# ReadAlongs/SoundSwallower

Hardware: AMD Instinct MI355X
Metric: senone-frames/sec (en-us PTM) (higher is better)
Workload: dtype f32+i32

## Files before the change

soundswallower_amd/csrc/ssw_host_active.inc:

```

static int
active_first_frames(const int32_t *sf, const int32_t *ef, int n_phones, int n_frames,
                    std::vector<int32_t> &first)
{
    first.assign((size_t)n_phones, INT_MAX);
    int32_t prev_first = 0, prev_last = 0;
    for (int i = 0; i < n_phones; ++i) {
        if (i > 0 && (sf[i] < sf[i - 1] || ef[i] < ef[i - 1])) {
            ssw_set_error("ssw_align_batch_active: phone windows must not decrease along an "
                          "utterance (phone %d); with such windows the reference's active set "
                          "depends on the path scores", i);
            return -1;
        }
        int32_t fi = i == 0 ? 0 : std::max(std::max((int32_t)1, sf[i]), prev_first);
        if (i > 0 && fi > prev_last)
            break;
        if (fi >= n_frames)
            break;
        first[i] = fi;
        prev_first = fi;
        prev_last = ef[i] < fi ? fi : ef[i];
    }
    return 0;
}
// ... 198 lines not shown
align_batch_active_impl(ssw_model_t *m, int scorer, const float *d_feats, int32_t n_utts,
                        const int32_t *frame_off, const int32_t *phone_off, const uint16_t *senid,
                        const int16_t *tmatid, const int32_t *sf, const int32_t *ef,
                        const uint32_t *seed_active, ssw_align_entry_t *state_io, int32_t *status,
                        int16_t *d_senscr, void *stream, const uint32_t *d_carry_rows)
{
    ModelBusy busy_(m);
    if (!busy_.ok)
        return -1;
    const ssw_host_model_t *h = m->h;
    hipStream_t st = (hipStream_t)stream;
    if (semi_refuse(scorer, "ssw_align_batch_active") < 0
        || cont_refuse(m, "ssw_align_batch_active") < 0)
        return -1;
    if (n_utts <= 0)
        return 0;
    if (check_scorer_shape(m, scorer) < 0)
        return -1;
    if (h->n_cb > 64 || h->n_emit_state != 3) {
        ssw_set_error("ssw_align_batch_active: built for <= 64 codebooks and 3-state HMMs");
        return -1;
    }
    if (h->cfg.ds != 1 || m->force_exact) {
        ssw_set_error("active-set batches: ds = 1 only");
        return -1;
    }
    if (!d_feats || !frame_off || !phone_off || !senid || !tmatid || !sf || !ef || !state_io
        || !status || frame_off[0] != 0 || phone_off[0] != 0) {
        ssw_set_error("ssw_align_batch_active: bad arguments");
        return -1;
    }
    HIP_OK(hipSetDevice(m->device));
    const int n_frames = frame_off[n_utts];
    std::vector<uint16_t> sen_slot((size_t)h->n_sen, 0);
    {
        std::vector<int> next((size_t)h->n_cb + 1, 0);
        for (int i = 0; i < h->n_sen; ++i)
            ++next[(size_t)h->sen2cb[i] + 1];
        for (int c = 0; c < h->n_cb; ++c)
            next[(size_t)c + 1] = next[(size_t)c] + ((next[(size_t)c + 1] + 3) & ~3);
        for (int i = 0; i < h->n_sen; ++i)
            sen_slot[(size_t)i] = (uint16_t)next[(size_t)h->sen2cb[i]]++;
    }
    std::vector<ActiveUtt> per_utt((size_t)n_utts);
    {
        ActiveJob J;
        J.h = h;
        J.sen_slot = sen_slot.data();
        J.n_utts = n_utts;
        J.frame_off = frame_off;
        J.phone_off = phone_off;
        J.sf = sf;
        J.ef = ef;
        J.senid = senid;
        J.seed_active = seed_active;
        J.out = per_utt.data();
        J.per_chunk = std::max(1, (n_utts + 4 * ssw_host_threads() - 1) / (4 * ssw_host_threads()));
        ssw_parallel_for((n_utts + J.per_chunk - 1) / J.per_chunk, active_build_chunk, &J);
    }
    std::vector<int32_t> seg_of_frame((size_t)std::max(n_frames, 1));
    std::vector<int32_t> seg_utt, seg_nreal, seg_boff(1, 0), utt_real_off((size_t)n_utts + 1, 0);
    std::vector<uint32_t> real_ent, bridge_ent;
    std::vector<uint16_t> real_rank;
    std::vector<unsigned long long> seg_cbmask;
    int cap = 1;
    for (int u = 0; u < n_utts; ++u) {
        const ActiveUtt &A = per_utt[(size_t)u];
        if (A.err != 0) {
            ssw_set_error("%s", A.msg);
            return -1;
        }
        const int f0 = frame_off[u], nf = frame_off[u + 1] - f0;
        utt_real_off[(size_t)u] = (int32_t)real_ent.size();
        real_ent.insert(real_ent.end(), A.real_ent.begin(), A.real_ent.end());
        real_rank.insert(real_rank.end(), A.real_rank.begin(), A.real_rank.end());
        utt_real_off[(size_t)u + 1] = (int32_t)real_ent.size();
        bridge_ent.insert(bridge_ent.end(), A.bridge_ent.begin(), A.bridge_ent.end());
        cap = std::max(cap, A.cap);
        for (size_t k = 0; k < A.seg_start.size(); ++k) {
            const int seg = (int)seg_utt.size();
            const int t0 = A.seg_start[k], t1 = k + 1 < A.seg_start.size() ? A.seg_start[k + 1] : nf;
// ... 86 lines not shown
```

soundswallower_amd/csrc/ssw_host_model.inc:

```

struct Knobs {
    int sen_fpb;
    int sen_r;
    int sen_groups;
    bool sen_generic;
    bool ms_senone_old;
    bool scan_fma;
    int mfma_min_frames;
    int score_piece;
    int host_pipe_cap;
    int mfma_steps;
    bool mfma_balance;
    int mfma_lds_pad;
    bool ptm_exact;
    bool frame_fused;
    int scan_audit;
    float selftest_eps_u;
    bool selftest_off;
    bool align_band, align_win;
    bool align_bt;
    char align_kernel[8];
    int align_band_tokens;
    int align_win_waves;
    bool align_timing;
    bool fp_band, fp_win;
    char fp_kernel[8];
    int fp_hist_band;
    int fp_big_tpb, fp_win_tpb;
    int fpa_sub;
};

static bool
knobs_dynamic()
{
    static const bool dyn = [] {
        const char *e = getenv("SSW_KNOBS_DYNAMIC");
        return e != NULL && e[0] == '1';
    }();
    return dyn;
}

static void
load_knobs(Knobs &k)
{
    auto env_int = [](const char *name, int dflt) {
        const char *e = getenv(name);
        return e != NULL ? atoi(e) : dflt;
    };
    auto env_is = [](const char *name, const char *val) {
        const char *e = getenv(name);
        return e != NULL && strcmp(e, val) == 0;
    };
    const char *e;
    e = getenv("SSW_SEN_FPB");
    k.sen_fpb = (e != NULL && (e[0] == '1' || e[0] == '2')) ? e[0] - '0' : 0;
    e = getenv("SSW_SEN_R");
    k.sen_r = (e != NULL && e[0] >= '1' && e[0] <= '4') ? e[0] - '0' : 0;
    e = getenv("SSW_SEN_GROUPS");
    k.sen_groups = e != NULL ? (atoi(e) > 0 ? atoi(e) : 0) : -1;
    k.sen_generic = getenv("SSW_SEN_GENERIC") != NULL;
    k.ms_senone_old = env_is("SSW_MS_SENONE", "old");
    k.scan_fma = env_is("SSW_SCAN", "fma");
    k.mfma_min_frames = env_int("SSW_MFMA_MIN_FRAMES", 1);
    k.fpa_sub = env_int("SSW_FPA_SUB", -1);
    k.score_piece = env_int("SSW_SCORE_PIECE", 16384) / 256 * 256;
    k.host_pipe_cap = std::max(2, env_int("SSW_HOST_PIPE_CAP", 16384) & ~1);
    e = getenv("SSW_MFMA_STEPS");
    k.mfma_steps = e != NULL ? (e[0] == '2' ? 2 : 1) : 0;
    e = getenv("SSW_MFMA_BALANCE");
    k.mfma_balance = !(e != NULL && e[0] == '0');
    k.mfma_lds_pad = env_int("SSW_MFMA_LDS_PAD", 0);
    e = getenv("SSW_PTM_EXACT");
    k.ptm_exact = e != NULL && e[0] == '1';
    k.frame_fused = getenv("SSW_FRAME_FUSED") != NULL;
    k.scan_audit = env_int("SSW_SCAN_AUDIT", 0);
    if (k.scan_audit < 0)
        k.scan_audit = 0;
    e = getenv("SSW_MFMA_SELFTEST_EPS");
    k.selftest_eps_u = e != NULL ? (float)atof(e) : 34.0f;
    k.selftest_off = env_is("SSW_MFMA_SELFTEST", "off");
    auto env_not0 = [](const char *name) {
        const char *v = getenv(name);
        return !(v != NULL && v[0] == '0');
    };
    auto env_str = [](const char *name, char (&dst)[8]) {
        const char *v = getenv(name);
        snprintf(dst, sizeof(dst), "%s", v != NULL ? v : "");
    };
    k.align_band = env_not0("SSW_ALIGN_BAND");
    k.align_win = env_not0("SSW_ALIGN_WIN");
    k.align_bt = env_not0("SSW_ALIGN_BT");
    env_str("SSW_ALIGN_KERNEL", k.align_kernel);
    k.align_band_tokens = env_int("SSW_ALIGN_BAND_TOKENS", 0);
// ... 47 lines not shown
    hipEvent_t ev[3];
    hipEvent_t ev_sc;

    uint32_t *cw() const { return topn_cw.as<uint32_t>(); }
    int4 *sc() const { return topn_sc.as<int4>(); }
    int *utt_off() const { return meta.as<int>(); }
    uint32_t *utt_start() const { return meta.as<uint32_t>() + ws_utts; }
};

struct ssw_model_s {
    ssw_host_model_t *h;
    Knobs kn;
    int scan_mode;
    int selftest_status;
    float selftest_worst_u, selftest_ms;
    char selftest_msg[200];
    int device;
    int n_cu;
    std::atomic<unsigned long long> owner;
    int owner_depth;
    int n_cbf, sen_stride;
    float *d_rec;
    float *d_rec28;
    float *d_recq;
    float *d_recmax;
    uint32_t *d_exlist;
    uint4 *d_wfrag;
    uint32_t *d_exlistm;
    int n_exact_form;
    uint8_t *d_mixw, *d_ms_pdf, *d_sen2cb, *d_logadd8, *d_logadd_mirror, *d_tp, *d_quad_cb;
    short4 *d_slot_sen;
    uint32_t *d_quad_info;
    uint16_t *d_sen_slot;
    DevBuf act_ws;
    int n_quads, slot_stride;
    int logadd_max;
    ScoreWs sw;
    DevBuf carry0;
    DevBuf carry_rows;
    unsigned char *h_stage[2];
    size_t h_stage_cap[2];
    hipEvent_t ev_stage[2];
    int stage_next;
    hipStream_t s_pipe, s_copy;
    hipEvent_t ev_piece[2], ev_down[2];
    unsigned char *h_pipe_feat[2], *h_pipe_out[2];
    float *d_pipe_feat[2];
    int16_t *d_pipe_out[2];
    size_t pipe_feat_cap, pipe_out_cap;
    int force_exact;
    int ms_raw;
    int64_t align_stats[2];
    int align_state_out_only;
    DevBuf feat_off;
    ssw_fe_tables_t *d_fe_tab;
    ssw_fe_config_t fe_tab_cfg;
    std::map<std::string, ssw_fe_rate_t *> *fe_rate_tab;
    int fe_nfilt, fe_noise;
    DevBuf fe_ws;
    hipEvent_t fe_ev[4];
    int fe_ev_ready, fe_timed;
    DevBuf align_ws;
    DevBuf fp_ws;
    hipStream_t s_up;
    hipEvent_t ev_up;
    uint64_t fp_ws_uid;
// ... 241 lines not shown
            HIP_OK(hipMemcpy(m->d_rec28, h->rec28, (size_t)ncbf * h->n_density * 28 * sizeof(float),
                             hipMemcpyHostToDevice));
            HIP_OK(hipMemcpy(m->d_exlistm, h->exlistm, nex * sizeof(uint32_t),
                             hipMemcpyHostToDevice));
        }
    }
    HIP_OK(hipMalloc((void **)&m->d_logadd8, 256));
    HIP_OK(hipMemcpy(m->d_logadd8, h->logadd8, 256, hipMemcpyHostToDevice));
    {
        int T = 0;
        for (int i = 0; i < 256; ++i)
            T = h->logadd8[i] > T ? h->logadd8[i] : T;
        m->logadd_max = T;
        std::vector<uint8_t> mir((size_t)3 * SSW_LOGADD_MIRROR);
        for (int part = 0; part < 2; ++part) {
            const int size = (part + 1) * SSW_LOGADD_MIRROR, mid = size / 2;
            uint8_t *out = mir.data() + (part ? SSW_LOGADD_MIRROR : 0);
            for (int e = 0; e < size; ++e) {
                const int d = e < mid ? mid - e : e - mid;
                out[e] = (uint8_t)(T - (d < 256 ? (int)h->logadd8[d] : 0));
            }
        }
        HIP_OK(hipMalloc((void **)&m->d_logadd_mirror, mir.size()));
        HIP_OK(hipMemcpy(m->d_logadd_mirror, mir.data(), mir.size(), hipMemcpyHostToDevice));
    }
    if (h->n_sen && h->sen2cb != NULL && h->cont_rec == NULL) {
        std::vector<uint8_t> s2c((size_t)h->n_sen);
        for (int i = 0; i < h->n_sen; ++i)
            s2c[i] = (uint8_t)h->sen2cb[i];
        HIP_OK(hipMalloc((void **)&m->d_sen2cb, s2c.size()));
        HIP_OK(hipMemcpy(m->d_sen2cb, s2c.data(), s2c.size(), hipMemcpyHostToDevice));
    }
    if ((h->ptm_mixw || h->ms_pdf) && h->sc_rec == NULL && h->cont_rec == NULL) {
        std::vector<int16_t> slot_sen;
        std::vector<uint8_t> quad_cb;
        for (int c = 0; c < h->n_cb; ++c) {
            size_t start = slot_sen.size();
            for (int i = 0; i < h->n_sen; ++i)
                if (h->sen2cb[i] == c)
                    slot_sen.push_back((int16_t)i);
            while ((slot_sen.size() - start) % 4)
                slot_sen.push_back(-1);
            for (size_t q = start / 4; q < slot_sen.size() / 4; ++q)
                quad_cb.push_back((uint8_t)c);
        }
        m->n_quads = (int)quad_cb.size();
        m->slot_stride = ((int)slot_sen.size() + 127) & ~127;
        m->sen_stride = m->slot_stride;
        const size_t rows = (size_t)h->n_feat * h->n_density;
        if (h->ptm_mixw) {
            std::vector<uint8_t> mw(rows * m->slot_stride, 0);
            for (size_t r = 0; r < rows; ++r)
                for (size_t sl = 0; sl < slot_sen.size(); ++sl) {
                    const int sen = slot_sen[sl] >= 0 ? slot_sen[sl] : slot_sen[sl & ~(size_t)3];
                    mw[r * m->slot_stride + sl] = h->ptm_mixw[r * h->n_sen + sen];
                }
            HIP_OK(hipMalloc((void **)&m->d_mixw, mw.size()));
            HIP_OK(hipMemcpy(m->d_mixw, mw.data(), mw.size(), hipMemcpyHostToDevice));
        }
        if (h->ms_pdf) {
            std::vector<uint8_t> mw(rows * m->slot_stride, 0);
            for (size_t sl = 0; sl < slot_sen.size(); ++sl) {
                const int sen = slot_sen[sl] >= 0 ? slot_sen[sl] : slot_sen[sl & ~(size_t)3];
                const uint8_t *src = h->ms_pdf + (size_t)sen * rows;
                for (size_t r = 0; r < rows; ++r)
                    mw[r * m->slot_stride + sl] = src[r];
            }
            HIP_OK(hipMalloc((void **)&m->d_ms_pdf, mw.size()));
            HIP_OK(hipMemcpy(m->d_ms_pdf, mw.data(), mw.size(), hipMemcpyHostToDevice));
        }
        {
            std::vector<uint32_t> qi(quad_cb.size());
            for (size_t q = 0; q < qi.size(); ++q) {
                const int16_t *sj = &slot_sen[4 * q];
                const bool run4 = sj[0] >= 0 && sj[1] == sj[0] + 1 && sj[2] == sj[0] + 2
                    && sj[3] == sj[0] + 3;
                qi[q] = ((uint32_t)sj[0] & 0xffffu) | ((uint32_t)run4 << 16)
                    | ((uint32_t)quad_cb[q] << 24);
            }
            HIP_OK(hipMalloc((void **)&m->d_quad_info, qi.size() * sizeof(uint32_t)));
            HIP_OK(hipMemcpy(m->d_quad_info, qi.data(), qi.size() * sizeof(uint32_t),
                             hipMemcpyHostToDevice));
        }
        HIP_OK(hipMalloc((void **)&m->d_quad_cb, quad_cb.size()));
        HIP_OK(hipMemcpy(m->d_quad_cb, quad_cb.data(), quad_cb.size(), hipMemcpyHostToDevice));
        {
            std::vector<uint16_t> sen_slot((size_t)h->n_sen, 0);
            for (size_t sl = 0; sl < slot_sen.size(); ++sl)
                if (slot_sen[sl] >= 0)
                    sen_slot[(size_t)slot_sen[sl]] = (uint16_t)sl;
            HIP_OK(hipMalloc((void **)&m->d_sen_slot, sen_slot.size() * sizeof(uint16_t) + 16));
            HIP_OK(hipMemcpy(m->d_sen_slot, sen_slot.data(), sen_slot.size() * sizeof(uint16_t),
                             hipMemcpyHostToDevice));
        }
        HIP_OK(hipMalloc((void **)&m->d_slot_sen, slot_sen.size() * sizeof(int16_t)));
        HIP_OK(hipMemcpy(m->d_slot_sen, slot_sen.data(), slot_sen.size() * sizeof(int16_t),
                         hipMemcpyHostToDevice));
    }
    if (h->tp) {
        size_t n = (size_t)h->tp_n_tmat * h->tp_n_state * (h->tp_n_state + 1);
        HIP_OK(hipMalloc((void **)&m->d_tp, n + 16));
        HIP_OK(hipMemcpy(m->d_tp, h->tp, n, hipMemcpyHostToDevice));
    }
    return 0;
}

static void
mfma_self_test(ssw_model_s *m)
{
    m->scan_mode = m->d_wfrag != NULL ? 1 : 0;
    m->selftest_status = 0;
    m->selftest_msg[0] = 0;
    if (m->d_wfrag == NULL || m->kn.selftest_off)
        return;
    {
        void *sym = NULL;
        if (hipGetSymbolAddress(&sym, HIP_SYMBOL(g_selftest_out)) != hipSuccess)
            (void)hipGetLastError();
    }
    const auto t0 = std::chrono::steady_clock::now();
    std::vector<float2> out((size_t)SSW_SELFTEST_TILES);
    hipLaunchKernelGGL(mfma_selftest_kernel, dim3(SSW_SELFTEST_TILES), dim3(64), 0, 0, 0x5eed2026u);
    hipError_t e = hipGetLastError();
    if (e == hipSuccess)
        e = hipMemcpyFromSymbol(out.data(), HIP_SYMBOL(g_selftest_out), sizeof(float2) * out.size());
    const float eps = m->kn.selftest_eps_u;
// ... 101 lines not shown
{
    if (m == NULL)
        return;
    ssw_feat_free(m->own_feat);
    if (m->device == SSW_DEVICE_NONE) {
        ssw_host_model_free(m->h);
        delete m;
        return;
    }
    (void)hipFree(m->featex_ws.p);
    (void)hipFree(m->d_rec);
    (void)hipFree(m->d_rec28);
    (void)hipFree(m->d_recq);
    (void)hipFree(m->d_recmax);
    (void)hipFree(m->d_exlist);
    (void)hipFree(m->d_wfrag);
    (void)hipFree(m->d_exlistm);
    (void)hipFree(m->align_ws.p);
    (void)hipFree(m->fp_ws.p);
    (void)hipFree(m->fpa_ws.p);
    (void)hipFree(m->gr_ws.p);
    (void)hipFree(m->text_scr.p);
    (void)hipFree(m->feat_off.p);
    (void)hipFree(m->d_fe_tab);
    if (m->fe_rate_tab)
        for (auto &kv : *m->fe_rate_tab)
            (void)hipFree(kv.second);
    delete m->fe_rate_tab;
    (void)hipFree(m->fe_ws.p);
    if (m->fe_ev_ready)
        for (int i = 0; i < 4; ++i)
            (void)hipEventDestroy(m->fe_ev[i]);
    (void)hipFree(m->d_sen_slot);
    (void)hipFree(m->act_ws.p);
    (void)hipFree(m->d_mixw);
    (void)hipFree(m->d_ms_pdf);
    (void)hipFree(m->d_sen2cb);
    if (m->s_up) {
        (void)hipEventDestroy(m->ev_up);
        (void)hipStreamDestroy(m->s_up);
    }
    (void)hipFree(m->d_quad_cb);
    (void)hipFree(m->d_quad_info);
    (void)hipFree(m->d_slot_sen);
    (void)hipFree(m->d_logadd8);
    (void)hipFree(m->d_logadd_mirror);
    (void)hipFree(m->d_tp);
    (void)hipFree(m->sw.topn_cw.p);
    (void)hipFree(m->sw.topn_sc.p);
    (void)hipFree(m->sw.meta.p);
    (void)hipFree(m->carry0.p);
    (void)hipFree(m->carry_rows.p);
    (void)hipFree(m->sw.d_nfixed);
    delete m->sw.utt_cache;
    delete m->sw.xcd_cuts;
    for (int k = 0; k < 2; ++k) {
        if (m->h_stage[k] != NULL) {
            (void)hipHostFree(m->h_stage[k]);
            (void)hipEventDestroy(m->ev_stage[k]);
        }
    }
    if (m->s_copy != NULL) {
        (void)hipStreamDestroy(m->s_copy);
        (void)hipStreamDestroy(m->s_pipe);
        for (int k = 0; k < 2; ++k) {
            (void)hipEventDestroy(m->ev_piece[k]);
// ... 119 lines not shown
```

soundswallower_amd/csrc/ssw_host_score.inc:

```
static int
ensure_score_ws(ssw_model_s *m, size_t rows, int n_utts)
{
    ScoreWs &w = m->sw;
    const uint64_t pairs = (uint64_t)rows * (uint64_t)m->n_cbf;
    if (pairs > 0xffffffffull) {
        ssw_set_error("batch of %d frames is too large (frames x codebooks x streams must fit 32 bits)",
                      (int)rows);
        return -1;
    }
    if (devbuf_reserve(w.topn_cw, sizeof(uint32_t) * (size_t)pairs, "ssw_score_batch") < 0
        || devbuf_reserve(w.topn_sc, sizeof(int4) * (size_t)pairs, "ssw_score_batch") < 0)
        return -1;
    if (w.d_nfixed == NULL) {
        if (dev_alloc(&w.d_nfixed, 4) < 0)
            return -1;
        HIP_OK(hipMemset(w.d_nfixed, 0, 4 * sizeof(unsigned long long)));
    }
    const size_t need_bits = 2 * ((rows + 31) / 32 + 2);
    if ((size_t)n_utts + 1 > w.ws_utts || need_bits > w.ws_bits) {
        const size_t wu = std::max((size_t)n_utts + 1, w.ws_utts_hint), wb = std::max(need_bits, w.ws_bits_hint);
        bool moved = false;
        w.ws_utts = w.ws_bits = 0;
        const int rc = devbuf_reserve(w.meta, sizeof(uint32_t) * (wu + wb), "ssw_score_batch", 0, &moved);
        if (moved && w.utt_cache)
// ... 129 lines not shown
    S.quad_info = m->d_quad_info;
    S.slot_sen = m->d_slot_sen;
    S.logadd8 = m->d_logadd8;
    S.logadd_mirror = m->d_logadd_mirror + (scorer == SSW_SCORER_MS ? SSW_LOGADD_MIRROR : 0);
    S.nfixed = move_stats ? m->sw.d_nfixed : NULL;
    S.nfixed_acc = m->sw.stats_accumulate;
    S.out = cp != NULL ? C.R.d_out : C.R.d_out + (size_t)lo * h->n_sen;
    if (cp != NULL) {
        S.utt_of_frame = cp->d_utt_of_frame;
        S.cutt_off = cp->d_frame_off;
        S.cstride = cp->d_cstride;
        S.crow_off = cp->d_crow_off;
        S.cpos = cp->d_cpos;
        S.frame_base = lo;
    }
    S.n_frames = n_frames;
    S.n_cb = h->n_cb;
    S.n_feat = h->n_feat;
    S.n_density = h->n_density;
    S.n_sen = h->n_sen;
    S.slot_stride = m->slot_stride;
    S.n_quads = m->n_quads;
    S.tab_max = m->logadd_max;
    if (scorer != SSW_SCORER_MS && 255 + SSW_MAX_NEG_ASCR + 3 * S.tab_max >= SSW_LOGADD_LDS) {
        ssw_set_error("unsupported log-add table (largest entry %d)", S.tab_max);
        return -1;
    }
    const bool ptm = scorer != SSW_SCORER_MS;
    const Knobs &kn = m->kn;
    int fpb = n_frames >= 4 * 512 ? 2 : 1;
    if (kn.sen_fpb != 0 && n_frames >= 4 * 512)
        fpb = kn.sen_fpb;
    size_t lds = 0;
    int R = (m->n_quads + SEN_MAX_THREADS - 1) / SEN_MAX_THREADS;
    const bool ms_packed = !ptm && ms_takes_packed_kernel(m, n_frames);
    if (cp != NULL && !ptm && !ms_packed) {
        ssw_set_error("internal error: compact rows asked of the un-packed ms senone kernel");
        return -1;
    }
    if ((ptm || ms_packed) && fpb == 2 && R < 4) {
        const int r7 = (m->n_quads + 447) / 448;
        R = r7 > R ? (r7 > 4 ? 4 : r7) : R;
    }
    if (kn.sen_r != 0)
        R = kn.sen_r;
    int threads = ((m->n_quads + R - 1) / R + 63) & ~63;
    if (threads < 256)
        threads = 256;
    if (threads > SEN_MAX_THREADS || (scorer == SSW_SCORER_MS && threads < m->n_cbf)) {
        ssw_set_error("unsupported senone/codebook shape (%d quads, %d codebook x stream)",
                      m->n_quads, m->n_cbf);
        return -1;
    }
    if (scorer == SSW_SCORER_MS && !ms_packed) {
        lds = 256 + 20 * (size_t)m->n_cbf + 16 * sizeof(int);
#define SSW_MS_LAUNCH(RR)                                                                    \
    if (h->n_feat == 3 && !kn.sen_generic)                                                   \
        hipLaunchKernelGGL((ms_senone_kernel<RR, 3>), dim3(n_frames), dim3(threads), lds, st, S); \
    else                                                                                     \
        hipLaunchKernelGGL((ms_senone_kernel<RR, 0>), dim3(n_frames), dim3(threads), lds, st, S)
        switch (R) {
        case 1: SSW_MS_LAUNCH(1); break;
        case 2: SSW_MS_LAUNCH(2); break;
        case 3: SSW_MS_LAUNCH(3); break;
        case 4: SSW_MS_LAUNCH(4); break;
        default:
            ssw_set_error("too many senones (%d quads)", m->n_quads);
            return -1;
        }
#undef SSW_MS_LAUNCH
        HIP_OK(hipGetLastError());
        return 0;
    }
    if (threads < fpb * m->n_cbf)
        fpb = 1;
    if (threads < m->n_cbf) {
        ssw_set_error("unsupported senone/codebook shape (%d quads, %d codebook x stream)",
                      m->n_quads, m->n_cbf);
        return -1;
    }
    lds = (ms_packed ? 2 * SSW_LOGADD_MIRROR : SSW_LOGADD_MIRROR)
        + 3 * 4 * (size_t)(ms_packed ? ((h->n_cb + 7) & ~7) : SSW_MAX_FEAT) * fpb + 16 * sizeof(int)
        + 2 * 32 * (size_t)m->n_cbf * fpb
        + 20 * (size_t)((fpb * m->n_cbf + 63) & ~63)
        + 8 * (size_t)R * threads + 16;
    const int n_units = (n_frames + fpb - 1) / fpb;
    int per_cu = 32 / (threads / 64);
    per_cu = per_cu < 1 ? 1 : per_cu;
    int groups = m->n_cu * per_cu;
    if ((C.R.flags & SSW_SCORE_SHARE_DEVICE) != 0 && groups < (n_units + 7) / 8)
        groups = (n_units + 7) / 8;
    if (kn.sen_groups >= 0)
        groups = kn.sen_groups > 0 ? kn.sen_groups : n_units;
    const dim3 grid(groups < n_units ? groups : n_units);
    const bool nf3 = h->n_feat == 3 && !kn.sen_generic;
    if (fpb != 1 && fpb != 2) {
        ssw_set_error("senone kernel: %d frames per group (1 or 2)", fpb);
        return -1;
    }
#define SSW_SEN_LAUNCH_C(RR, FP, NFV, MSV, CV)                                               \
    hipLaunchKernelGGL((ptm_senone_kernel<4, RR, FP, NFV, MSV, CV>), grid, dim3(threads), lds, st, S)
#define SSW_SEN_LAUNCH_NF(RR, FP, MSV, CV)                                                   \
    if (nf3)                                                                                 \
        SSW_SEN_LAUNCH_C(RR, FP, 3, MSV, CV);                                                \
    else                                                                                     \
        SSW_SEN_LAUNCH_C(RR, FP, 0, MSV, CV)
#define SSW_SEN_LAUNCH_FP(RR, MSV, CV)                                                       \
    if (fpb == 2) {                                                                          \
        SSW_SEN_LAUNCH_NF(RR, 2, MSV, CV);                                                   \
    } else {                                                                                 \
        SSW_SEN_LAUNCH_NF(RR, 1, MSV, CV);                                                   \
    }
#define SSW_SEN_LAUNCH(RR)                                                                   \
    if (ms_packed && cp != NULL) {                                                           \
        SSW_SEN_LAUNCH_FP(RR, true, true);                                                   \
    } else if (ms_packed) {                                                                  \
        SSW_SEN_LAUNCH_FP(RR, true, false);                                                  \
    } else if (cp != NULL) {                                                                 \
// ... 937 lines not shown
```

soundswallower_amd/csrc/ssw_k1b_senone.inc:

```

struct SenoneParams {
    const uint32_t *topn_cw;
    const int4 *topn_sc;
    const uint8_t *mixw;
    const uint8_t *quad_cb;
    const short4 *slot_sen;
    const uint32_t *quad_info;
    const uint8_t *logadd8;
    const uint8_t *logadd_mirror;
    unsigned long long *nfixed;
    int16_t *out;
    int n_frames, n_cb, n_feat, n_density, n_sen, slot_stride, n_quads;
    int aw, zero;
    int raw;
    int tab_max;
    const int32_t *utt_of_frame, *cutt_off, *cstride;
    const long long *crow_off;
    const uint32_t *cpos;
    int nfixed_acc;
    int frame_base;
};

constexpr int SEN_MAX_THREADS = 1024;

#define SSW_LOGADD_LDS 512
#define SSW_LOGADD_MIRROR 1024

__device__ __forceinline__ int
fast_logadd(int x, int y, const uint8_t *tab)
{
    const int hi = x > y ? x : y;
    const int r = x < y ? x : y;
    return r - (int)tab[hi - r];
}

typedef unsigned short ushort2v __attribute__((ext_vector_type(2)));
typedef uint32_t uint2u __attribute__((ext_vector_type(2), aligned(2)));

__device__ __forceinline__ uint32_t
pk_min_u16(uint32_t a, uint32_t b)
{
    return __builtin_bit_cast(uint32_t, __builtin_elementwise_min(__builtin_bit_cast(ushort2v, a),
                                                                  __builtin_bit_cast(ushort2v, b)));
}

__device__ __forceinline__ uint32_t
pk_max_u16(uint32_t a, uint32_t b)
{
    return __builtin_bit_cast(uint32_t, __builtin_elementwise_max(__builtin_bit_cast(ushort2v, a),
                                                                  __builtin_bit_cast(ushort2v, b)));
}

template <int HI>
__device__ __forceinline__ uint32_t
pk_add_bcast_u16(uint32_t a, uint32_t b)
{
    uint32_t r;
    if (HI)
        asm("v_pk_add_u16 %0, %1, %2 op_sel:[0,1] op_sel_hi:[1,1]" : "=v"(r) : "v"(a), "v"(b));
    else
        asm("v_pk_add_u16 %0, %1, %2 op_sel:[0,0] op_sel_hi:[1,0]" : "=v"(r) : "v"(a), "v"(b));
    return r;
}

template <int NS, int TOPN, int MID>
__device__ __forceinline__ void
quad_chains(const uint32_t (*mw)[TOPN], const uint2 *np, uint32_t (&acc)[2])
{
    constexpr int NC = 2 * NS;
    uint32_t x2[NC];
// ... 138 lines not shown
}

template <int TOPN, int R, int FPB, int NF, bool MS, bool COMPACT = false>
__global__ void __launch_bounds__(SEN_MAX_THREADS) __attribute__((amdgpu_waves_per_eu(8, 8)))
ptm_senone_kernel(SenoneParams P)
{
    constexpr int MIRROR = MS ? 2 * SSW_LOGADD_MIRROR : SSW_LOGADD_MIRROR;
    constexpr int MID = MIRROR / 2;
    constexpr int MS_NMAX = 640;
#ifdef SSW_TIMELINE_SEN
#define STL(k)                                                                               \
    if ((threadIdx.x & 63) == 0) {                                                           \
        int wv = blockIdx.x * 11 + (threadIdx.x >> 6);                                       \
        if (wv < 16384)                                                                      \
            g_timeline[wv * 6 + (k)] = __builtin_amdgcn_s_memtime();                        \
    }
#else
#define STL(k)
#endif
    STL(0)
    __builtin_amdgcn_s_setprio(3);
    const int n_feat = NF ? NF : P.n_feat;
    static_assert(TOPN == 4, "top-N block is packed 4 x 8 bit");
    extern __shared__ __align__(16) unsigned char smem[];
    const int n_cbf = P.n_cb * P.n_feat;
    uint8_t *s_tab = smem;
    const int NORM_W = MS ? ((P.n_cb + 7) & ~7) : SSW_MAX_FEAT;
    int *s_norm = reinterpret_cast<int *>(smem + MIRROR);
    int *s_red = s_norm + 3 * NORM_W * FPB;
    uint4 *s_item = reinterpret_cast<uint4 *>(s_red + 16);
    const int n_item_pad = (FPB * n_cbf + 63) & ~63;
    int4 *s_stage_sc = reinterpret_cast<int4 *>(s_item + 2 * 2 * n_cbf * FPB);
    uint32_t *s_stage_cw = reinterpret_cast<uint32_t *>(s_stage_sc + n_item_pad);
    short4 *s_sen4 = reinterpret_cast<short4 *>(s_stage_cw + n_item_pad);

    const int tid = threadIdx.x;
    const int nthr = blockDim.x;
    const uint32_t T = (uint32_t)P.tab_max;
    const int n_units = (P.n_frames + FPB - 1) / FPB;
    const int stride_u = (int)gridDim.x;
    int u = (int)blockIdx.x;
    if (u >= n_units)
        return;

    if ((uint32_t)(uintptr_t)(__attribute__((address_space(3))) unsigned char *)smem != 0u)
        __builtin_trap();

    uint32_t my_a, my_b;
    {
        int fr = 0;
#pragma unroll
        for (int k = 1; k < FPB; ++k)
            fr += tid >= k * n_cbf ? 1 : 0;
        const int i = tid - fr * n_cbf, f = i % n_feat;
        const int nidx = MS ? fr * NORM_W + i / n_feat : fr * SSW_MAX_FEAT + f;
        my_a = (uint32_t)fr | (uint32_t)nidx << 4 | (uint32_t)(f * P.n_density) << 16;
        my_b = (uint32_t)(2 * (i * FPB + fr));
    }
    int4 sc0 = make_int4(0, 0, 0, 0);
    uint32_t cw0 = 0;
    auto item_live = [&](int unit) {
        return tid < FPB * n_cbf && unit * FPB + (int)(my_a & 0xfu) < P.n_frames;
    };
    auto fetch_item = [&](int unit) {
        if (item_live(unit)) {
            sc0 = P.topn_sc[(size_t)unit * FPB * n_cbf + tid];
            cw0 = P.topn_cw[(size_t)unit * FPB * n_cbf + tid];
// ... 46 lines not shown
                    q = q > MS_NMAX ? MS_NMAX : q;
                } else {
                    q = -((v[k] >> SSW_SENSCR_SHIFT) - norm);
                    q = q > SSW_MAX_NEG_ASCR ? SSW_MAX_NEG_ASCR : q;
                }
                const uint32_t e = (uint32_t)(q & 0x3ff) + (k > 1 ? T * (uint32_t)(k - 1) : 0u);
                sp[k] = e;
            }
            const uint32_t e0 = MS ? 0u : sp[0];
#pragma unroll
            for (int k = 0; k < TOPN; ++k)
                sp[k] -= e0;
            if (MS) {
                const int a0 = -norm - (int)(3u * T) * n_feat;
                if (a0 < 0 || a0 > 30000)
                    atomicOr(&s_red[12 + ns], 1 << (int)(my_a & 0xfu));
            }
            uint4 *dst = s_item + (2 * buf * n_cbf * FPB + (int)my_b);
            const uint32_t row0 = my_a >> 16;
            dst[0] = make_uint4(__umul24(row0 + (cw0 & 0xffu), (uint32_t)P.slot_stride),
                                __umul24(row0 + ((cw0 >> 8) & 0xffu), (uint32_t)P.slot_stride),
                                __umul24(row0 + ((cw0 >> 16) & 0xffu), (uint32_t)P.slot_stride),
                                __umul24(row0 + (cw0 >> 24), (uint32_t)P.slot_stride));
            reinterpret_cast<uint2 *>(dst + 1)[0]
                = make_uint2(sp[0] | (sp[1] << 16), sp[2] | (sp[3] << 16));
            reinterpret_cast<uint32_t *>(dst + 1)[2] = MS
                ? (uint32_t)((-norm - (int)(3u * T) * n_feat) & 0xffff) * 0x10001u
                : e0 * 0x10001u;
        }
    };

    fetch_item(u);
    uint32_t qi_ld[R];
    short4 sen4_ld[R];
#pragma unroll
    for (int r = 0; r < R; ++r) {
        const int q = r * nthr + tid;
        qi_ld[r] = q < P.n_quads ? P.quad_info[q] : 0u;
        sen4_ld[r] = q < P.n_quads ? P.slot_sen[q] : make_short4(-1, -1, -1, -1);
    }
    constexpr int TAB_DW = MIRROR / 4;
    uint32_t tv[(TAB_DW + 255) / 256] = {};
#pragma unroll
    for (int j = 0; j < (TAB_DW + 255) / 256; ++j) {
        const int e = tid + j * nthr;
        if (e < TAB_DW)
            tv[j] = reinterpret_cast<const uint32_t *>(P.logadd_mirror)[e];
    }
    if (tid < 3 * NORM_W * FPB)
        s_norm[tid] = MS ? 0 : SSW_WORST_SCORE;
    if (3 * NORM_W * FPB > nthr)
        for (int i = tid + nthr; i < 3 * NORM_W * FPB; i += nthr)
            s_norm[i] = MS ? 0 : SSW_WORST_SCORE;
    if (tid < 16)
        s_red[tid] = tid < 12 ? INT_MAX : 0;
    if (P.nfixed != nullptr && blockIdx.x == 0 && tid == 0) {
        P.nfixed[1] = (P.nfixed_acc ? P.nfixed[1] : 0ull) + P.nfixed[0];
        P.nfixed[0] = 0ull;
    }
    lds_barrier();
    norm_item(u, 0);
#pragma unroll
    for (int j = 0; j < (TAB_DW + 255) / 256; ++j)
        if (tid + j * nthr < TAB_DW)
            reinterpret_cast<uint32_t *>(s_tab)[tid + j * nthr] = tv[j];
    lds_barrier();
    stage_item(u, 0, 0);

    const __amdgpu_buffer_rsrc_t mw_rsrc = __builtin_amdgcn_make_buffer_rsrc(
        const_cast<uint8_t *>(P.mixw)
            + (uint32_t)__builtin_amdgcn_readfirstlane((int)((uint32_t)tid & ~63u) * 4),
        (short)4, 64, (int)(1u << 23));
    uint32_t qoff[R];
#pragma unroll
    for (int r = 0; r < R; ++r) {
        const int q = r * nthr + tid;
        const uint32_t qi = qi_ld[r];
        qoff[r] = (qi >> 24) * (uint32_t)(n_feat * FPB * 32) | ((qi >> 16) & 1u);
        s_sen4[q] = sen4_ld[r];
    }

    for (int it = 0;; ++it) {
        const int t0 = u * FPB;
        const int nfr = (P.n_frames - t0) < FPB ? (P.n_frames - t0) : FPB;
        const int u_next = u + stride_u;
        const bool has_next = u_next < n_units;
        const int buf = it & 1, slot = it % 3, slot_next = (it + 1) % 3;
        lds_barrier();
        if (has_next)
            fetch_item_dma(u_next);
        STL(1)
        uint32_t asc2[R][FPB][2];
        const uint4 *item_b = s_item + 2 * buf * n_cbf * FPB;
#pragma unroll
        for (int r = 0; r < R; ++r) {
            const int q = r * nthr + tid;
            const int soff = __builtin_amdgcn_readfirstlane(r * nthr * 4);
#pragma unroll
            for (int fr = 0; fr < FPB; ++fr) {
                const uint32_t dead = (q < P.n_quads && fr < nfr) ? 0u : 0xffffffffu;
                asc2[r][fr][0] = asc2[r][fr][1] = dead;
            }
            if (q < P.n_quads) {
                const uint4 *item_cb = reinterpret_cast<const uint4 *>(
                    reinterpret_cast<const unsigned char *>(item_b) + (qoff[r] & ~1u));
                if (MS) {
#pragma unroll
                    for (int fr = 0; fr < FPB; ++fr)
                        if (fr < nfr)
                            asc2[r][fr][0] = asc2[r][fr][1]
                                = reinterpret_cast<const uint32_t *>(item_cb + 2 * fr + 1)[2];
                }
#pragma unroll
                for (int fr = 0; fr < FPB; ++fr) {
                    {
                        constexpr int NI = R * FPB;
                        const int item = r * FPB + fr;
                        if (item * 4 < NI)
                            __builtin_amdgcn_s_setprio(3);
                        else if (item * 4 < 2 * NI)
                            __builtin_amdgcn_s_setprio(2);
                        else if (item * 4 < 3 * NI)
                            __builtin_amdgcn_s_setprio(1);
                        else
                            __builtin_amdgcn_s_setprio(0);
                    }
                    if (fr < nfr) {
                        if (NF) {
                            uint32_t mw[NF ? NF : 1][TOPN];
                            uint2 np[NF ? NF : 1];
                            uint32_t zsum = 0;
#pragma unroll
                            for (int f = 0; f < NF; ++f) {
                                const uint4 ro = item_cb[2 * (f * FPB + fr)];
                                const uint4 sc4 = item_cb[2 * (f * FPB + fr) + 1];
                                np[f] = make_uint2(sc4.x, sc4.y);
                                if (!MS)
                                    zsum += sc4.z;
// ... 1 lines not shown
                                mw[f][1] = (uint32_t)__builtin_amdgcn_raw_buffer_load_b32(mw_rsrc, (int)ro.y, soff, 0);
                                mw[f][2] = (uint32_t)__builtin_amdgcn_raw_buffer_load_b32(mw_rsrc, (int)ro.z, soff, 0);
                                mw[f][3] = (uint32_t)__builtin_amdgcn_raw_buffer_load_b32(mw_rsrc, (int)ro.w, soff, 0);
                            }
                            if (!MS) {
                                asc2[r][fr][0] += zsum;
                                asc2[r][fr][1] += zsum;
                            }
                            quad_chains<NF ? NF : 1, TOPN, MID>(mw, np, asc2[r][fr]);
                        } else
                        for (int f = 0; f < n_feat; ++f) {
                            const uint4 ro = item_cb[2 * (f * FPB + fr)];
                            const uint4 sc4 = item_cb[2 * (f * FPB + fr) + 1];
                            const uint2 np = make_uint2(sc4.x, sc4.y);
                            if (!MS) {
                                asc2[r][fr][0] += sc4.z;
                                asc2[r][fr][1] += sc4.z;
                            }
                            uint32_t mw[1][TOPN];
                            mw[0][0] = (uint32_t)__builtin_amdgcn_raw_buffer_load_b32(mw_rsrc, (int)ro.x, soff, 0);
                            mw[0][1] = (uint32_t)__builtin_amdgcn_raw_buffer_load_b32(mw_rsrc, (int)ro.y, soff, 0);
                            mw[0][2] = (uint32_t)__builtin_amdgcn_raw_buffer_load_b32(mw_rsrc, (int)ro.z, soff, 0);
                            mw[0][3] = (uint32_t)__builtin_amdgcn_raw_buffer_load_b32(mw_rsrc, (int)ro.w, soff, 0);
                            quad_chains<1, TOPN, MID>(mw, &np, asc2[r][fr]);
                        }
                    }
                }
            }
        }
        STL(2)
        __builtin_amdgcn_s_setprio(3);
        if (has_next)
            take_item_dma(u_next);
        short4 sen4[R];
#pragma unroll
        for (int r = 0; r < R; ++r)
            sen4[r] = s_sen4[r * nthr + tid];
        int c_utt[FPB];
        uint4 c_pos[R][FPB];
        if (COMPACT) {
#pragma unroll
            for (int fr = 0; fr < FPB; ++fr) {
                c_utt[fr] = fr < nfr
                    ? __builtin_amdgcn_readfirstlane(P.utt_of_frame[P.frame_base + t0 + fr]) : 0;
#pragma unroll
                for (int r = 0; r < R; ++r) {
                    const int q = r * nthr + tid;
                    c_pos[r][fr] = (q < P.n_quads && fr < nfr)
                        ? *reinterpret_cast<const uint4 *>(P.cpos + (size_t)c_utt[fr] * P.slot_stride + 4 * q)
                        : make_uint4(0xffffffffu, 0xffffffffu, 0xffffffffu, 0xffffffffu);
                }
            }
        }
#pragma unroll
        for (int fr = 0; fr < FPB; ++fr) {
            uint32_t b2 = 0xffffffffu;
#pragma unroll
            for (int r = 0; r < R; ++r)
                b2 = pk_min_u16(b2, pk_min_u16(asc2[r][fr][0], asc2[r][fr][1]));
            const int lo = (int)(b2 & 0xffffu), hi = (int)(b2 >> 16);
            const int wmin = -wave_max_dpp(-(lo < hi ? lo : hi));
            if ((tid & 63) == 0)
                atomicMin(&s_red[slot * FPB + fr], wmin);
        }
        if (has_next)
            norm_item(u_next, slot_next);
        lds_barrier();
        int best[FPB];
#pragma unroll
        for (int fr = 0; fr < FPB; ++fr)
// ... 10 lines not shown
                    const int stride = __builtin_amdgcn_readfirstlane(P.cstride[uu]);
                    const long long ro = P.crow_off[uu]
                        + (long long)(P.frame_base + t0 + fr
                                      - __builtin_amdgcn_readfirstlane(P.cutt_off[uu])) * stride;
                    const uintptr_t rb = reinterpret_cast<uintptr_t>(P.out + ro);
                    const uint32_t rb_lo = (uint32_t)__builtin_amdgcn_readfirstlane((int)(uint32_t)rb);
                    const uint32_t rb_hi = (uint32_t)__builtin_amdgcn_readfirstlane((int)(uint32_t)(rb >> 32));
                    const __amdgpu_buffer_rsrc_t orsrc = __builtin_amdgcn_make_buffer_rsrc(
                        reinterpret_cast<void *>(((uintptr_t)rb_hi << 32) | rb_lo), (short)0,
                        stride * 2, 0x00020000);
                    const uint32_t b2 = (uint32_t)best[fr] * 0x10001u;
#pragma unroll
                    for (int r = 0; r < R; ++r) {
                        const uint32_t lo2 = asc2[r][fr][0] - b2, hi2 = asc2[r][fr][1] - b2;
                        const uint4 cp = c_pos[r][fr];
                        if (cp.x != 0xffffffffu)
                            __builtin_amdgcn_raw_buffer_store_b16((short)(lo2 & 0xffffu), orsrc, (int)cp.x, 0, 0);
                        if (cp.y != 0xffffffffu)
                            asm volatile("buffer_store_short_d16_hi %0, %1, %2, 0 offen"
                                         :: "v"(lo2), "v"(cp.y), "s"(orsrc) : "memory");
                        if (cp.z != 0xffffffffu)
                            __builtin_amdgcn_raw_buffer_store_b16((short)(hi2 & 0xffffu), orsrc, (int)cp.z, 0, 0);
                        if (cp.w != 0xffffffffu)
                            asm volatile("buffer_store_short_d16_hi %0, %1, %2, 0 offen"
                                         :: "v"(hi2), "v"(cp.w), "s"(orsrc) : "memory");
                    }
                }
            }
        } else
#pragma unroll
        for (int r = 0; r < R; ++r) {
            const int q = r * nthr + tid;
            if (q < P.n_quads) {
                const bool run4 = qoff[r] & 1u;
                const int sj[4] = { sen4[r].x, sen4[r].y, sen4[r].z, sen4[r].w };
#pragma unroll
                for (int fr = 0; fr < FPB; ++fr) {
                    if (fr < nfr) {
                        const uint32_t b2 = (uint32_t)best[fr] * 0x10001u;
                        int16_t *orow = P.out + (size_t)(t0 + fr) * P.n_sen;
                        uint2u pk;
                        pk.x = asc2[r][fr][0] - b2;
                        pk.y = asc2[r][fr][1] - b2;
                        if (run4) {
                            *reinterpret_cast<uint2u *>(orow + sj[0]) = pk;
                        } else {
                            const int16_t v[4] = { (int16_t)(pk.x & 0xffffu), (int16_t)(pk.x >> 16),
                                                   (int16_t)(pk.y & 0xffffu), (int16_t)(pk.y >> 16) };
#pragma unroll
                            for (int j = 0; j < 4; ++j)
                                if (sj[j] >= 0)
                                    orow[sj[j]] = v[j];
                        }
                    }
                }
            }
        }
        STL(4)
        if (MS && marked != 0) {
            for (int fr = 0; fr < nfr; ++fr)
                if ((marked >> fr) & 1)
                    ms_exact_frame<R, COMPACT>(P, t0 + fr, tid, nthr, reinterpret_cast<int *>(s_stage_cw));
        }
        if (!has_next)
            break;
        stage_item(u_next, slot_next, buf ^ 1);
        if (tid < NORM_W * FPB)
            s_norm[slot * NORM_W * FPB + tid] = MS ? 0 : SSW_WORST_SCORE;
        if (tid < FPB)
            s_red[slot_next * FPB + tid] = INT_MAX;
        u = u_next;
    }
#undef STL
}

struct SenoneFrameParams {
    const uint32_t *topn_cw;
    const int4 *topn_sc;
    const uint8_t *mixw, *quad_cb, *logadd8;
    unsigned long long cb_mask[4];
    const uint32_t *sen_bits;
    const short4 *slot_sen;
    int16_t *out;
    int16_t *raw;
    int n_cb, n_feat, n_density, n_sen, slot_stride, n_quads;
// ... 469 lines not shown
```

soundswallower_amd/csrc/ssw_kernels.hip:

```cpp
#pragma clang fp contract(off)

#include <hip/hip_runtime.h>

#include <algorithm>
#include <array>
#include <atomic>
#include <functional>
#include <map>
#include <memory>
#include <set>
#include <chrono>
#include <climits>
#include <cmath>
#include <cstdint>
#include <cstdio>
#include <cstdlib>
#include <cstring>
#include <string>
#include <thread>
#include <vector>

#include "ssw_internal.h"

#define HIP_OK(expr)                                                                         \
// ... 1 lines not shown
        hipError_t e_ = (expr);                                                              \
        if (e_ != hipSuccess) {                                                              \
            ssw_set_error("%s failed: %s (%s:%d)", #expr, hipGetErrorString(e_), __FILE__,   \
                          __LINE__);                                                         \
            return -1;                                                                       \
        }                                                                                    \
    } while (0)

namespace {
#include "ssw_dev_common.inc"
#include "ssw_k1a_chain.inc"
#include "ssw_k1a_frames.inc"
#include "ssw_top5_select.inc"
#include "ssw_k1a_mfma.inc"
#include "ssw_k1b_senone.inc"
#include "ssw_k4_feat.inc"
#include "ssw_align_common.inc"
#include "ssw_k2_align.inc"
#include "ssw_k2_anytopo.inc"
#include "ssw_search_common.inc"
#include "ssw_k5_firstpass.inc"
#include "ssw_k6_compact.inc"
#include "ssw_k7_fpactive.inc"
#include "ssw_k8_fe.inc"
#include "ssw_k9_grammar.inc"
#include "ssw_k10_semi.inc"
#include "ssw_k11_cont.inc"
#include "ssw_k12_feat.inc"

}

#include "ssw_ws_layout.inc"
#include "ssw_xcd_cut.inc"
#include "ssw_feat_tiles.inc"
#include "ssw_host_model.inc"
#include "ssw_host_semi.inc"
static int cont_check_shape(const ssw_model_s *m, int scorer);
static int cont_refuse(const ssw_model_s *m, const char *who);
static int cont_launch(ssw_model_s *m, const float *d_feats, int32_t n_frames, int16_t *d_out,
                       hipStream_t st);
#include "ssw_host_score.inc"
#include "ssw_host_align.inc"
#include "ssw_host_compact.inc"
#include "ssw_host_active.inc"
#include "ssw_host_mgau.inc"
#include "ssw_host_search.inc"
#include "ssw_host_feat.inc"
#include "ssw_host_fe.inc"
#include "ssw_host_firstpass.inc"
#include "ssw_host_fpactive.inc"
#include "ssw_host_grammar.inc"
#include "ssw_host_devmem.inc"
#include "ssw_host_comm.inc"
#include "ssw_host_cont.inc"
#include "ssw_host_featex.inc"
```

Measured before the change: 67.19 million.

## Use prefix-run slot layout so senone quads store contiguous partial runs directly

Senone slots are now laid out so each quad holds a contiguous run of senone ids, padding only at breaks. The run length and starting byte offset are packed into quad_info and qoff, so most quads write their outputs with 8-, 4- or 2-byte stores instead of scattered per-senone stores. The per-block LDS copy of slot_sen is removed; the few irregular quads reload slot_sen from global memory. The prefix layout is used only when it does not raise R or the thread count, and the host slot map is now computed once at model load instead of on every active-set batch.

Result: faster. 68.14 million (median of 6 runs) (+1.4%).

```diff
diff --git a/soundswallower_amd/csrc/ssw_host_active.inc b/soundswallower_amd/csrc/ssw_host_active.inc
--- a/soundswallower_amd/csrc/ssw_host_active.inc
+++ b/soundswallower_amd/csrc/ssw_host_active.inc
@@ -254,21 +254,12 @@
     }
     HIP_OK(hipSetDevice(m->device));
     const int n_frames = frame_off[n_utts];
-    std::vector<uint16_t> sen_slot((size_t)h->n_sen, 0);
-    {
-        std::vector<int> next((size_t)h->n_cb + 1, 0);
-        for (int i = 0; i < h->n_sen; ++i)
-            ++next[(size_t)h->sen2cb[i] + 1];
-        for (int c = 0; c < h->n_cb; ++c)
-            next[(size_t)c + 1] = next[(size_t)c] + ((next[(size_t)c + 1] + 3) & ~3);
-        for (int i = 0; i < h->n_sen; ++i)
-            sen_slot[(size_t)i] = (uint16_t)next[(size_t)h->sen2cb[i]]++;
-    }
+    const uint16_t *sen_slot = m->h_sen_slot;
     std::vector<ActiveUtt> per_utt((size_t)n_utts);
     {
         ActiveJob J;
         J.h = h;
-        J.sen_slot = sen_slot.data();
+        J.sen_slot = sen_slot;
         J.n_utts = n_utts;
         J.frame_off = frame_off;
         J.phone_off = phone_off;
diff --git a/soundswallower_amd/csrc/ssw_host_model.inc b/soundswallower_amd/csrc/ssw_host_model.inc
--- a/soundswallower_amd/csrc/ssw_host_model.inc
+++ b/soundswallower_amd/csrc/ssw_host_model.inc
@@ -4,6 +4,7 @@
     int sen_r;
     int sen_groups;
     bool sen_generic;
+    bool slot_dense;
     bool ms_senone_old;
     bool scan_fma;
     int mfma_min_frames;
@@ -59,6 +60,7 @@
     e = getenv("SSW_SEN_GROUPS");
     k.sen_groups = e != NULL ? (atoi(e) > 0 ? atoi(e) : 0) : -1;
     k.sen_generic = getenv("SSW_SEN_GENERIC") != NULL;
+    k.slot_dense = env_is("SSW_SLOT_LAYOUT", "dense");
     k.ms_senone_old = env_is("SSW_MS_SENONE", "old");
     k.scan_fma = env_is("SSW_SCAN", "fma");
     k.mfma_min_frames = env_int("SSW_MFMA_MIN_FRAMES", 1);
@@ -172,6 +174,8 @@
     short4 *d_slot_sen;
     uint32_t *d_quad_info;
     uint16_t *d_sen_slot;
+    uint16_t *h_sen_slot;
+    int slot_prefix;
     DevBuf act_ws;
     int n_quads, slot_stride;
     int logadd_max;
@@ -479,18 +483,18 @@
         HIP_OK(hipMemcpy(m->d_sen2cb, s2c.data(), s2c.size(), hipMemcpyHostToDevice));
     }
     if ((h->ptm_mixw || h->ms_pdf) && h->sc_rec == NULL && h->cont_rec == NULL) {
-        std::vector<int16_t> slot_sen;
-        std::vector<uint8_t> quad_cb;
-        for (int c = 0; c < h->n_cb; ++c) {
-            size_t start = slot_sen.size();
-            for (int i = 0; i < h->n_sen; ++i)
-                if (h->sen2cb[i] == c)
-                    slot_sen.push_back((int16_t)i);
-            while ((slot_sen.size() - start) % 4)
-                slot_sen.push_back(-1);
-            for (size_t q = start / 4; q < slot_sen.size() / 4; ++q)
-                quad_cb.push_back((uint8_t)c);
-        }
+        SlotLayout lay = slot_layout(h->sen2cb, h->n_sen, h->n_cb, false);
+        m->slot_prefix = 0;
+        if (!m->kn.slot_dense) {
+            SlotLayout pre = slot_layout(h->sen2cb, h->n_sen, h->n_cb, true);
+            if (slot_layout_prefix_fits((int)lay.quad_cb.size(), (int)pre.quad_cb.size(),
+                                        SEN_MAX_THREADS)) {
+                lay = std::move(pre);
+                m->slot_prefix = 1;
+            }
+        }
+        const std::vector<int16_t> &slot_sen = lay.slot_sen;
+        const std::vector<uint8_t> &quad_cb = lay.quad_cb;
         m->n_quads = (int)quad_cb.size();
         m->slot_stride = ((int)slot_sen.size() + 127) & ~127;
         m->sen_stride = m->slot_stride;
@@ -519,11 +523,9 @@
         {
             std::vector<uint32_t> qi(quad_cb.size());
             for (size_t q = 0; q < qi.size(); ++q) {
-                const int16_t *sj = &slot_sen[4 * q];
-                const bool run4 = sj[0] >= 0 && sj[1] == sj[0] + 1 && sj[2] == sj[0] + 2
-                    && sj[3] == sj[0] + 3;
-                qi[q] = ((uint32_t)sj[0] & 0xffffu) | ((uint32_t)run4 << 16)
-                    | ((uint32_t)quad_cb[q] << 24);
+                const uint32_t n = lay.quad_n[q];
+                qi[q] = ((uint32_t)lay.quad_s0[q] & 0xffffu) | ((uint32_t)(n == 4) << 16)
+                    | (n << 17) | ((uint32_t)quad_cb[q] << 24);
             }
             HIP_OK(hipMalloc((void **)&m->d_quad_info, qi.size() * sizeof(uint32_t)));
             HIP_OK(hipMemcpy(m->d_quad_info, qi.data(), qi.size() * sizeof(uint32_t),
@@ -539,6 +541,12 @@
             HIP_OK(hipMalloc((void **)&m->d_sen_slot, sen_slot.size() * sizeof(uint16_t) + 16));
             HIP_OK(hipMemcpy(m->d_sen_slot, sen_slot.data(), sen_slot.size() * sizeof(uint16_t),
                              hipMemcpyHostToDevice));
+            m->h_sen_slot = (uint16_t *)malloc(sen_slot.size() * sizeof(uint16_t));
+            if (m->h_sen_slot == NULL) {
+                ssw_set_error("out of memory");
+                return -1;
+            }
+            memcpy(m->h_sen_slot, sen_slot.data(), sen_slot.size() * sizeof(uint16_t));
         }
         HIP_OK(hipMalloc((void **)&m->d_slot_sen, slot_sen.size() * sizeof(int16_t)));
         HIP_OK(hipMemcpy(m->d_slot_sen, slot_sen.data(), slot_sen.size() * sizeof(int16_t),
@@ -706,6 +714,7 @@
         for (int i = 0; i < 4; ++i)
             (void)hipEventDestroy(m->fe_ev[i]);
     (void)hipFree(m->d_sen_slot);
+    free(m->h_sen_slot);
     (void)hipFree(m->act_ws.p);
     (void)hipFree(m->d_mixw);
     (void)hipFree(m->d_ms_pdf);
diff --git a/soundswallower_amd/csrc/ssw_host_score.inc b/soundswallower_amd/csrc/ssw_host_score.inc
--- a/soundswallower_amd/csrc/ssw_host_score.inc
+++ b/soundswallower_amd/csrc/ssw_host_score.inc
@@ -185,21 +185,14 @@
     if (kn.sen_fpb != 0 && n_frames >= 4 * 512)
         fpb = kn.sen_fpb;
     size_t lds = 0;
-    int R = (m->n_quads + SEN_MAX_THREADS - 1) / SEN_MAX_THREADS;
     const bool ms_packed = !ptm && ms_takes_packed_kernel(m, n_frames);
     if (cp != NULL && !ptm && !ms_packed) {
         ssw_set_error("internal error: compact rows asked of the un-packed ms senone kernel");
         return -1;
     }
-    if ((ptm || ms_packed) && fpb == 2 && R < 4) {
-        const int r7 = (m->n_quads + 447) / 448;
-        R = r7 > R ? (r7 > 4 ? 4 : r7) : R;
-    }
-    if (kn.sen_r != 0)
-        R = kn.sen_r;
-    int threads = ((m->n_quads + R - 1) / R + 63) & ~63;
-    if (threads < 256)
-        threads = 256;
+    const SenoneShape shape = senone_shape(m->n_quads, fpb, ptm || ms_packed, kn.sen_r,
+                                           SEN_MAX_THREADS);
+    const int R = shape.R, threads = shape.threads;
     if (threads > SEN_MAX_THREADS || (scorer == SSW_SCORER_MS && threads < m->n_cbf)) {
         ssw_set_error("unsupported senone/codebook shape (%d quads, %d codebook x stream)",
                       m->n_quads, m->n_cbf);
@@ -236,7 +229,7 @@
         + 3 * 4 * (size_t)(ms_packed ? ((h->n_cb + 7) & ~7) : SSW_MAX_FEAT) * fpb + 16 * sizeof(int)
         + 2 * 32 * (size_t)m->n_cbf * fpb
         + 20 * (size_t)((fpb * m->n_cbf + 63) & ~63)
-        + 8 * (size_t)R * threads + 16;
+        + 16;
     const int n_units = (n_frames + fpb - 1) / fpb;
     int per_cu = 32 / (threads / 64);
     per_cu = per_cu < 1 ? 1 : per_cu;
diff --git a/soundswallower_amd/csrc/ssw_k1b_senone.inc b/soundswallower_amd/csrc/ssw_k1b_senone.inc
--- a/soundswallower_amd/csrc/ssw_k1b_senone.inc
+++ b/soundswallower_amd/csrc/ssw_k1b_senone.inc
@@ -36,6 +36,7 @@
 
 typedef unsigned short ushort2v __attribute__((ext_vector_type(2)));
 typedef uint32_t uint2u __attribute__((ext_vector_type(2), aligned(2)));
+typedef uint32_t uint1u __attribute__((aligned(2)));
 
 __device__ __forceinline__ uint32_t
 pk_min_u16(uint32_t a, uint32_t b)
@@ -240,7 +241,6 @@
     const int n_item_pad = (FPB * n_cbf + 63) & ~63;
     int4 *s_stage_sc = reinterpret_cast<int4 *>(s_item + 2 * 2 * n_cbf * FPB);
     uint32_t *s_stage_cw = reinterpret_cast<uint32_t *>(s_stage_sc + n_item_pad);
-    short4 *s_sen4 = reinterpret_cast<short4 *>(s_stage_cw + n_item_pad);
 
     const int tid = threadIdx.x;
     const int nthr = blockDim.x;
@@ -353,12 +353,10 @@
 
     fetch_item(u);
     uint32_t qi_ld[R];
-    short4 sen4_ld[R];
 #pragma unroll
     for (int r = 0; r < R; ++r) {
         const int q = r * nthr + tid;
         qi_ld[r] = q < P.n_quads ? P.quad_info[q] : 0u;
-        sen4_ld[r] = q < P.n_quads ? P.slot_sen[q] : make_short4(-1, -1, -1, -1);
     }
     constexpr int TAB_DW = MIRROR / 4;
     uint32_t tv[(TAB_DW + 255) / 256] = {};
@@ -395,10 +393,8 @@
     uint32_t qoff[R];
 #pragma unroll
     for (int r = 0; r < R; ++r) {
-        const int q = r * nthr + tid;
         const uint32_t qi = qi_ld[r];
-        qoff[r] = (qi >> 24) * (uint32_t)(n_feat * FPB * 32) | ((qi >> 16) & 1u);
-        s_sen4[q] = sen4_ld[r];
+        qoff[r] = (qi >> 24) * (uint32_t)(n_feat * FPB * 32) | ((qi >> 17) & 7u) | (qi << 17);
     }
 
     for (int it = 0;; ++it) {
@@ -424,7 +420,7 @@
             }
             if (q < P.n_quads) {
                 const uint4 *item_cb = reinterpret_cast<const uint4 *>(
-                    reinterpret_cast<const unsigned char *>(item_b) + (qoff[r] & ~1u));
+                    reinterpret_cast<const unsigned char *>(item_b) + (qoff[r] & 0x1ffe0u));
                 if (MS) {
 #pragma unroll
                     for (int fr = 0; fr < FPB; ++fr)
@@ -492,10 +488,6 @@
         __builtin_amdgcn_s_setprio(3);
         if (has_next)
             take_item_dma(u_next);
-        short4 sen4[R];
-#pragma unroll
-        for (int r = 0; r < R; ++r)
-            sen4[r] = s_sen4[r * nthr + tid];
         int c_utt[FPB];
         uint4 c_pos[R][FPB];
         if (COMPACT) {
@@ -572,25 +564,54 @@
         for (int r = 0; r < R; ++r) {
             const int q = r * nthr + tid;
             if (q < P.n_quads) {
-                const bool run4 = qoff[r] & 1u;
-                const int sj[4] = { sen4[r].x, sen4[r].y, sen4[r].z, sen4[r].w };
+                uint32_t qo = qoff[r];
+                asm volatile("" : "+v"(qo));
+                const uint32_t n = qo & 7u;
+                const uint32_t boff = (qo >> 16) & 0xfffeu;
+                uint2u pk[FPB];
+                unsigned char *orow[FPB];
 #pragma unroll
                 for (int fr = 0; fr < FPB; ++fr) {
-                    if (fr < nfr) {
-                        const uint32_t b2 = (uint32_t)best[fr] * 0x10001u;
-                        int16_t *orow = P.out + (size_t)(t0 + fr) * P.n_sen;
-                        uint2u pk;
-                        pk.x = asc2[r][fr][0] - b2;
-                        pk.y = asc2[r][fr][1] - b2;
-                        if (run4) {
-                            *reinterpret_cast<uint2u *>(orow + sj[0]) = pk;
-                        } else {
-                            const int16_t v[4] = { (int16_t)(pk.x & 0xffffu), (int16_t)(pk.x >> 16),
-                                                   (int16_t)(pk.y & 0xffffu), (int16_t)(pk.y >> 16) };
+                    const uint32_t b2 = (uint32_t)best[fr] * 0x10001u;
+                    pk[fr].x = asc2[r][fr][0] - b2;
+                    pk[fr].y = asc2[r][fr][1] - b2;
+                    orow[fr] = reinterpret_cast<unsigned char *>(P.out + (size_t)(t0 + fr) * P.n_sen);
+                }
+                if (n == 4) {
+#pragma unroll
+                    for (int fr = 0; fr < FPB; ++fr)
+                        if (fr < nfr)
+                            *reinterpret_cast<uint2u *>(orow[fr] + boff) = pk[fr];
+                } else if (n != 0) {
+                    if (n & 2u) {
+#pragma unroll
+                        for (int fr = 0; fr < FPB; ++fr)
+                            if (fr < nfr)
+                                *reinterpret_cast<uint1u *>(orow[fr] + boff) = pk[fr].x;
+                    }
+                    if (n & 1u) {
+                        const uint32_t boff1 = boff + 2 * (n & 2u);
+#pragma unroll
+                        for (int fr = 0; fr < FPB; ++fr)
+                            if (fr < nfr)
+                                *reinterpret_cast<uint16_t *>(orow[fr] + boff1)
+                                    = (uint16_t)(((n & 2u) ? pk[fr].y : pk[fr].x) & 0xffffu);
+                    }
+                } else {
+                    uint32_t lane = (uint32_t)tid;
+                    asm volatile("" : "+v"(lane));
+                    const short4 s4 = P.slot_sen[(uint32_t)(r * nthr) + lane];
+                    const int sj[4] = { s4.x, s4.y, s4.z, s4.w };
+#pragma unroll
+                    for (int fr = 0; fr < FPB; ++fr) {
+                        if (fr < nfr) {
+                            const int16_t v[4]
+                                = { (int16_t)(pk[fr].x & 0xffffu), (int16_t)(pk[fr].x >> 16),
+                                    (int16_t)(pk[fr].y & 0xffffu), (int16_t)(pk[fr].y >> 16) };
 #pragma unroll
                             for (int j = 0; j < 4; ++j)
                                 if (sj[j] >= 0)
-                                    orow[sj[j]] = v[j];
+                                    reinterpret_cast<int16_t *>(orow[fr])[sj[j]] = v[j];
                         }
                     }
                 }
diff --git a/soundswallower_amd/csrc/ssw_kernels.hip b/soundswallower_amd/csrc/ssw_kernels.hip
--- a/soundswallower_amd/csrc/ssw_kernels.hip
+++ b/soundswallower_amd/csrc/ssw_kernels.hip
@@ -57,6 +57,7 @@
 
 #include "ssw_ws_layout.inc"
 #include "ssw_xcd_cut.inc"
+#include "ssw_slot_layout.inc"
 #include "ssw_feat_tiles.inc"
 #include "ssw_host_model.inc"
 #include "ssw_host_semi.inc"
diff --git a/soundswallower_amd/csrc/ssw_slot_layout.inc b/soundswallower_amd/csrc/ssw_slot_layout.inc
--- /dev/null
+++ b/soundswallower_amd/csrc/ssw_slot_layout.inc
@@ -0,0 +1,84 @@
+#include <cstddef>
+#include <cstdint>
+#include <vector>
+
+struct SlotLayout {
+    std::vector<int16_t> slot_sen;
+    std::vector<uint8_t> quad_cb;
+    std::vector<int16_t> quad_s0;
+    std::vector<uint8_t> quad_n;
+};
+
+static inline SlotLayout
+slot_layout(const int16_t *sen2cb, int n_sen, int n_cb, bool prefix)
+{
+    SlotLayout L;
+    for (int c = 0; c < n_cb; ++c) {
+        const size_t start = L.slot_sen.size();
+        int prev = -2;
+        for (int i = 0; i < n_sen; ++i) {
+            if (sen2cb[i] != c)
+                continue;
+            if (prefix && i != prev + 1)
+                while (L.slot_sen.size() % 4)
+                    L.slot_sen.push_back(-1);
+            L.slot_sen.push_back((int16_t)i);
+            prev = i;
+        }
+        while (L.slot_sen.size() % 4)
+            L.slot_sen.push_back(-1);
+        for (size_t q = start / 4; q < L.slot_sen.size() / 4; ++q)
+            L.quad_cb.push_back((uint8_t)c);
+    }
+    const size_t n_quads = L.quad_cb.size();
+    L.quad_s0.resize(n_quads);
+    L.quad_n.resize(n_quads);
+    for (size_t q = 0; q < n_quads; ++q) {
+        const int16_t *sj = &L.slot_sen[4 * q];
+        int n = 1;
+        while (n < 4 && sj[n] == sj[0] + n)
+            ++n;
+        bool form = true;
+        for (int j = n; j < 4; ++j)
+            form = form && sj[j] < 0;
+        L.quad_s0[q] = sj[0];
+        L.quad_n[q] = (uint8_t)(form ? n : 0);
+    }
+    return L;
+}
+
+struct SenoneShape {
+    int R, threads;
+};
+
+static inline SenoneShape
+senone_shape(int n_quads, int fpb, bool seven_waves, int force_r, int max_threads)
+{
+    SenoneShape s;
+    s.R = (n_quads + max_threads - 1) / max_threads;
+    if (seven_waves && fpb == 2 && s.R < 4) {
+        const int r7 = (n_quads + 447) / 448;
+        s.R = r7 > s.R ? (r7 > 4 ? 4 : r7) : s.R;
+    }
+    if (force_r != 0)
+        s.R = force_r;
+    if (s.R < 1)
+        s.R = 1;
+    s.threads = ((n_quads + s.R - 1) / s.R + 63) & ~63;
+    if (s.threads < 256)
+        s.threads = 256;
+    return s;
+}
+
+static inline bool
+slot_layout_prefix_fits(int dense_quads, int prefix_quads, int max_threads)
+{
+    for (int fpb = 1; fpb <= 2; ++fpb)
+        for (int seven = 0; seven < 2; ++seven) {
+            const SenoneShape d = senone_shape(dense_quads, fpb, seven != 0, 0, max_threads);
+            const SenoneShape p = senone_shape(prefix_quads, fpb, seven != 0, 0, max_threads);
+            if (p.R > d.R || p.threads > d.threads)
+                return false;
+        }
+    return true;
+}
```
